# jungmannlab/picasso

Measured on AMD Instinct MI355X. Metric: localizations/sec (7x7 ROI, MLE), higher is better.
Workload: dtype f32+f64; 1 GPU; 10000-frame 512x512 uint16 simulated DNA-PAINT movie per GPU, 1001675 spots per GPU, 7x7 ROI MLE (sigmaxy), identify+cut+fit+table resident in HBM; frames=10000, height=512, width=512, box=7, max_it=100, localizations_total=1001675, mle_mode=refit, refit_spots_rank0=7346, frame_ranges_in_flight=2, all_gather=none

## Files before the change

picasso_amd/csrc/gausslq.hip:

```cpp
#include <algorithm>
#include <cstdlib>
#include <cstring>

#include "lq_common.h"

#pragma clang fp contract(off)

namespace pmi {
namespace lq {

#ifndef LQ_SBUF_PAD
#define LQ_SBUF_PAD 0
#endif
__host__ __device__ constexpr size_t lq_sbuf_doubles(int m) { return (size_t)6 * (size_t)((m + 1) & ~1) + LQ_SBUF_PAD; }
__device__ __forceinline__ void grp_sync()
{
    __builtin_amdgcn_wave_barrier();
    __threadfence_block();
    __builtin_amdgcn_wave_barrier();
}
template <int GS, int E>
__device__ __forceinline__ void rows_to_lds(const double (&v)[E], int lane, int m, double *buf)
{
#pragma unroll
// ... 721 lines not shown
    const int64_t src = (int64_t)blockIdx.x * blockDim.x + threadIdx.x;
    if (src >= n) return;
    const int64_t i = src + (d_row0 ? *d_row0 : 0);
    const float *t = th + src * 6;
    ((uint32_t *)cols.c[0])[i] = (uint32_t)frame[src];
    ((float *)cols.c[1])[i] = (float)((double)t[0] + (double)x[src]);
    ((float *)cols.c[2])[i] = (float)((double)t[1] + (double)y[src]);
    ((float *)cols.c[3])[i] = t[2];
    ((float *)cols.c[4])[i] = t[4];
    ((float *)cols.c[5])[i] = t[5];
    ((float *)cols.c[6])[i] = t[3];
    ((float *)cols.c[7])[i] = lq_precision(t[2], t[4], t[5], t[3], em);
    ((float *)cols.c[8])[i] = lq_precision(t[2], t[5], t[4], t[3], em);
    const float a = np_maxf(t[4], t[5]), b = np_minf(t[4], t[5]);
    ((float *)cols.c[9])[i] = (a - b) / a;
    ((float *)cols.c[10])[i] = ng[src];
}

}

int identify_impl(const void *d_movie, int dtype, int64_t F, int64_t Y, int64_t X, int box, double min_ng,
                  const int64_t *roi4, int64_t f_lo, int64_t f_hi, int64_t label_offset,
                  int32_t *d_frame, int32_t *d_y, int32_t *d_x, float *d_ng, int64_t cap, int64_t *d_out_n,
                  bool defer_exact, hipStream_t s);

}

extern "C" {

int pmi_gausslq_set_mode(int mode)
{
    using namespace pmi;
    if (mode != PMI_LQ_FAST && mode != PMI_LQ_REFIT && mode != PMI_LQ_STRICT) { set_error("unknown gausslq mode %d", mode); return PMI_ERR_ARG; }
    lq::g_lq_mode = mode;
    return PMI_OK;
}

int pmi_gausslq_get_mode(int *mode)
{
    if (mode) *mode = pmi::lq::lq_mode_now();
    return PMI_OK;
}

int pmi_gausslq_last_refit_count(int64_t *n_refit)
{
    unsigned h[16];
    const int rc = pmi::lq::g_lq_stats.read(h);
// ... 77 lines not shown
int pmi_localize_lq_dev(const void *d_movie, int dtype, int64_t F, int64_t Y, int64_t X, int box, double min_ng,
                        const int64_t *roi4, int64_t f_lo, int64_t f_hi, double baseline, double sensitivity,
                        double gain, int em, void *d_table, int64_t cap, int64_t *d_out_n, void *stream)
{
    using namespace pmi;
    if (cap <= 0) { set_error("capacity must be positive"); return PMI_ERR_ARG; }
    int rc = lq::check_box(box);
    if (rc != PMI_OK) return rc;
    struct Ids { int32_t *f, *y, *x; float *ng, *th; };
    auto carve = [=](void *ptr) {
        Ids d;
        d.f = (int32_t *)ptr; d.y = d.f + cap; d.x = d.y + cap;
        d.ng = (float *)(d.x + cap);
        d.th = d.ng + cap;
        return d;
    };
    lq::LqCols cols;
    for (int c = 0; c < PMI_LQ_COLUMNS; c++) cols.c[c] = (char *)d_table + (size_t)c * cap * 4;
    FusedRanges fr;
    fr.ids_bytes = (size_t)cap * (16 + 6 * 4);
    fr.capc = cap;
    fr.cap = cap;
    fr.rejects = false;
    fr.scan = [&](void *ids, int64_t lo, int64_t hi, int64_t *d_cnt, hipStream_t st) {
        const Ids d = carve(ids);
        return identify_impl(d_movie, dtype, F, Y, X, box, min_ng, roi4, lo, hi, 0, d.f, d.y, d.x, d.ng, cap, d_cnt, false, st);
    };
    fr.fit = [&](void *ids, const int64_t *d_rows, int range, hipStream_t st) {
        const Ids d = carve(ids);
        return lq::fit_movie(d_movie, dtype, Y, X, d.f, d.y, d.x, cap, d_rows, box, baseline, sensitivity, gain, d.th, nullptr,
                             nullptr, range, st);
    };
    fr.table = [&](void *ids, const int64_t *d_rows, const int64_t *d_row0, hipStream_t st) {
        const Ids d = carve(ids);
        hipLaunchKernelGGL(lq::locs_from_fits_lq_kernel, dim3((unsigned)((cap + 255) / 256)), dim3(256), 0, st, d.f, d.y, d.x, d.ng,
                           d.th, cap, d_rows, em, cols, d_row0);
        PMI_HIP(hipGetLastError());
        return PMI_OK;
    };
    return fused_ranges(fr, 1, F, Y, X, f_lo, f_hi, d_out_n, (hipStream_t)stream);
}

}
```

picasso_amd/csrc/gaussmle.hip:

```cpp
#include <algorithm>
#include <cmath>
#include <cstdlib>
#include <cstring>
#include <vector>

#include "fit_common.h"

namespace pmi {

__device__ __forceinline__ unsigned borderline(float D, int kk, float eps_lo, float eps_hi)
{
    const float wide = fmaxf(1.0f, (float)(kk - 1) * FIT_MARGIN_GROWTH);
    const float epsf = 0.5f * (eps_lo + eps_hi), epsm = 0.5f * (eps_hi - eps_lo) * wide;
    return ((D >= epsf - epsm && D < epsf + epsm) ? FLAG_MARGIN : 0u) | (kk > FIT_SLOW_ITERATIONS ? FLAG_SLOW : 0u);
}
struct StepHistory { float prev, prev2, wprev; int run; };
__device__ __forceinline__ bool wobbles(float st, float value, int kk, StepHistory &h)
{
    const float w = kk >= 3 ? (st - 2.0f * h.prev) + h.prev2 : 0.0f;
    const bool wob = w * h.wprev < 0.0f && fabsf(w) > FIT_WOBBLE_RATIO * fabsf(h.wprev) && fabsf(w) > FIT_WOBBLE_FLOOR * fabsf(value);
    h.run = wob ? h.run + 1 : 0;
    h.wprev = w; h.prev2 = h.prev; h.prev = st;
    return h.run >= FIT_WOBBLE_RUN || (h.run >= 2 && kk >= FIT_WOBBLE_LATE);
}
// ... 545 lines not shown
}

static int mle_mode_now()
{
    static const char *env = getenv("PMI_MLE_MODE");
    if (env) {
        if (!strcmp(env, "fast")) return PMI_MLE_FAST;
        if (!strcmp(env, "strict")) return PMI_MLE_STRICT;
        if (!strcmp(env, "refit")) return PMI_MLE_REFIT;
    }
    return g_mle_mode;
}
static int mle_libm_now()
{
    static const char *env = getenv("PMI_MLE_LIBM");
    if (env) {
        if (!strcmp(env, "auto")) return PMI_LIBM_AUTO;
        if (!strcmp(env, "glibc")) return PMI_LIBM_GLIBC;
        if (!strcmp(env, "device")) return PMI_LIBM_DEVICE;
    }
    return g_mle_libm;
}

int fit_impl(FitParams p, int method, bool from_movie, int range, hipStream_t s)
{
    if (p.box < 3 || p.box > PMI_MAX_BOX || (p.box & 1) == 0) { set_error("box must be odd, 3..%d (got %d)", PMI_MAX_BOX, p.box); return PMI_ERR_ARG; }
    if (method != PMI_MLE_SIGMA && method != PMI_MLE_SIGMAXY) { set_error("Method not available."); return PMI_ERR_ARG; }
    if (p.N < 0) { set_error("negative N"); return PMI_ERR_ARG; }
    if (p.N == 0) return PMI_OK;
    if (p.N > 0x7fffffffLL) { set_error("too many spots for one call"); return PMI_ERR_ARG; }
    const int g_cu_count = device_cu_count();
    const int mode = mle_mode_now();
    const int64_t BATCH = FIT_BATCH;
    const int64_t nb = (p.N + BATCH - 1) / BATCH;
    void *ptr = nullptr, *fptr = nullptr;
    int rc;
    if ((rc = scratch(SCR_FIT, (size_t)nb * 40 + 64, &ptr)) != PMI_OK) return rc;
    const size_t per_batch = (size_t)std::min<int64_t>(p.N, BATCH);
    const size_t acc_blocks = (per_batch + ACC_BLOCK - 1) / ACC_BLOCK + 2;
    if ((rc = scratch(SCR_STAGE_D, per_batch * (FISHER_STRIDE * sizeof(double) + 12 * sizeof(float) + 3 * sizeof(int32_t) + 1) + acc_blocks * sizeof(unsigned) + 32, &fptr)) != PMI_OK) return rc;
    float *state = reinterpret_cast<float *>((char *)fptr + per_batch * FISHER_STRIDE * sizeof(double));
    int32_t *flag_list = reinterpret_cast<int32_t *>(state + per_batch * 12);
    int32_t *unstable_list = flag_list + per_batch;
    int32_t *acc_list = unstable_list + per_batch;
    unsigned *acc_blk = reinterpret_cast<unsigned *>(acc_list + per_batch);
    unsigned char *refit_mark = reinterpret_cast<unsigned char *>(acc_blk + acc_blocks);
    unsigned long long *queues = (unsigned long long *)ptr;
// ... 38 lines not shown
        if (p.refit_mark && !g8) PMI_HIP(hipMemsetAsync(refit_mark, 0, (size_t)(p.N - p.first), s));
        const int64_t count = p.N - p.first;
        const int64_t blocks = std::min<int64_t>((count + FIT_WAVES - 1) / FIT_WAVES, (int64_t)g_cu_count * 8);
        const dim3 grid((unsigned)std::max<int64_t>(blocks, 1));
        auto wave_per_spot = [&](int stages) {
            p.queue = queues + 3 * bi + (stages == FIT_STAGE_FINAL ? (p.final_list ? 2 : 1) : 0);
            if (method == PMI_MLE_SIGMAXY) {
                if (from_movie) launch_fit_ppl<6, true>(ppl, grid, s, p, stages); else launch_fit_ppl<6, false>(ppl, grid, s, p, stages);
            } else {
                if (from_movie) launch_fit_ppl<5, true>(ppl, grid, s, p, stages); else launch_fit_ppl<5, false>(ppl, grid, s, p, stages);
            }
        };
        if (mode != PMI_MLE_STRICT && g8 && from_movie && cut) {
            FitParams pi = p;
            pi.spots_out = cut;
            launch_fit_g8(pi, method, true, g_cu_count, state, FIT_STAGE_INIT_ONLY, s);
            PMI_HIP(hipGetLastError());
            FitParams q = p;
            q.spots = cut - p.first * (int64_t)(p.box * p.box);
            if (p.ng_io) {
                int32_t *al = nb == 1 && p.alist_out ? p.alist_out : acc_list;
                unsigned *ab = nb == 1 && p.alist_out ? p.alist_blk_out : acc_blk;
                if ((rc = build_accept_list(p.accept, p.first, p.N, p.d_n, ab, al, s)) != PMI_OK) return rc;
                q.alist = al;
                q.alist_n = ab + (count + ACC_BLOCK - 1) / ACC_BLOCK;
            }
            launch_fit_g8(q, method, false, g_cu_count, state, FIT_STAGE_ITERATE_ONLY, s);
            PMI_HIP(hipGetLastError());
            if (mode == PMI_MLE_REFIT)
                launch_fit_strict(q, method, false, flag_list, q.flag_count, count, g_cu_count, s);
            PMI_HIP(hipGetLastError());
            launch_fit_g8(q, method, false, g_cu_count, state, FIT_STAGE_FINAL, s);
        } else {
        if (mode == PMI_MLE_STRICT) {
            FitParams ps = p;
            ps.libm_glibc = libm_all;
            launch_fit_strict(ps, method, from_movie, nullptr, nullptr, count, g_cu_count, s);
        } else {
            if (g8) launch_fit_g8(p, method, from_movie, g_cu_count, state, FIT_STAGE_NEWTON, s);
            else wave_per_spot(FIT_STAGE_NEWTON);
            PMI_HIP(hipGetLastError());
            if (mode == PMI_MLE_REFIT)
                launch_fit_strict(p, method, from_movie, flag_list, p.flag_count, count, g_cu_count, s);
        }
        PMI_HIP(hipGetLastError());
        if (g8) launch_fit_g8(p, method, from_movie, g_cu_count, state, FIT_STAGE_FINAL, s);
// ... 81 lines not shown
    ((uint32_t *)cols.c[0])[i] = (uint32_t)frame[src];
    ((float *)cols.c[1])[i] = (float)((double)t[0] + (double)x[src] - (double)off);
    ((float *)cols.c[2])[i] = (float)((double)t[1] + (double)y[src] - (double)off);
    ((float *)cols.c[3])[i] = t[2];
    ((float *)cols.c[4])[i] = t[4];
    ((float *)cols.c[5])[i] = t[5];
    ((float *)cols.c[6])[i] = t[3];
    ((float *)cols.c[7])[i] = sqrtf(c[0]);
    ((float *)cols.c[8])[i] = sqrtf(c[1]);
    float a = np_maxf(t[4], t[5]), b = np_minf(t[4], t[5]);
    ((float *)cols.c[9])[i] = (a - b) / a;
    ((float *)cols.c[10])[i] = ng[src];
    ((float *)cols.c[11])[i] = ll[src];
    ((uint32_t *)cols.c[12])[i] = (uint32_t)it[src];
    ((float *)cols.c[13])[i] = sqrtf(c[2]);
    ((float *)cols.c[14])[i] = sqrtf(c[3]);
    ((float *)cols.c[15])[i] = sqrtf(c[4]);
    ((float *)cols.c[16])[i] = sqrtf(c[5]);
}

int identify_impl(const void *d_movie, int dtype, int64_t F, int64_t Y, int64_t X, int box, double min_ng,
                  const int64_t *roi4, int64_t f_lo, int64_t f_hi, int64_t label_offset,
                  int32_t *d_frame, int32_t *d_y, int32_t *d_x, float *d_ng, int64_t cap, int64_t *d_out_n,
                  bool defer_exact, hipStream_t s);

}

extern "C" {

int pmi_mle_set_mode(int mode, double margin)
{
    using namespace pmi;
    if (mode != PMI_MLE_FAST && mode != PMI_MLE_REFIT && mode != PMI_MLE_STRICT) { set_error("unknown MLE mode %d", mode); return PMI_ERR_ARG; }
    if (!(margin >= 0.0 && margin < 1.0)) { set_error("margin must lie in [0, 1)"); return PMI_ERR_ARG; }
    g_mle_mode = mode;
    g_mle_margin = margin;
    return PMI_OK;
}

int pmi_mle_set_libm(int which)
{
    using namespace pmi;
    if (which != PMI_LIBM_DEVICE && which != PMI_LIBM_GLIBC && which != PMI_LIBM_AUTO) { set_error("unknown libm %d", which); return PMI_ERR_ARG; }
    g_mle_libm = which;
    return PMI_OK;
}

// ... 194 lines not shown
    int64_t cy0 = 0, cx0 = 0, cy1 = Y, cx1 = X;
    if (roi4) { cy0 = roi4[0]; cx0 = roi4[1]; cy1 = roi4[2]; cx1 = roi4[3]; }
    struct Ids { int32_t *f, *y, *x; float *ng, *th, *cr, *ll; int32_t *it, *tlist; unsigned *blk; unsigned char *acc; };
    const size_t acc_blocks = (size_t)((capc + ACC_BLOCK - 1) / ACC_BLOCK) + 2;
    const int nblk_c = (int)((capc + ACC_BLOCK - 1) / ACC_BLOCK);
    auto carve = [=](void *ptr) {
        Ids d;
        d.f = (int32_t *)ptr; d.y = d.f + capc; d.x = d.y + capc;
        d.ng = (float *)(d.x + capc);
        d.th = d.ng + capc; d.cr = d.th + capc * 6; d.ll = d.cr + capc * 6;
        d.it = (int32_t *)(d.ll + capc);
        d.tlist = d.it + capc;
        d.blk = (unsigned *)(d.tlist + capc);
        d.acc = (unsigned char *)(d.blk + acc_blocks);
        return d;
    };
    LocCols lc;
    for (int c = 0; c < PMI_LOC_COLUMNS; c++) lc.c[c] = (char *)d_table + (size_t)c * cap * 4;
    FusedRanges fr;
    fr.ids_bytes = (size_t)capc * (16 + 15 * 4 + 1) + acc_blocks * sizeof(unsigned) + 16;
    fr.capc = capc;
    fr.cap = cap;
    fr.rejects = defer;
    fr.scan = [&](void *ids, int64_t lo, int64_t hi, int64_t *d_cnt, hipStream_t st) {
        const Ids d = carve(ids);
        return identify_impl(d_movie, dtype, F, Y, X, box, min_ng, roi4, lo, hi, 0, d.f, d.y, d.x, d.ng, capc, d_cnt, defer, st);
    };
    fr.fit = [&](void *ids, const int64_t *d_rows, int range, hipStream_t st) {
        const Ids d = carve(ids);
        FitParams p = {};
        p.movie = d_movie; p.dtype = dtype; p.Y = Y; p.X = X; p.frame = d.f; p.y = d.y; p.x = d.x;
        p.baseline = (float)baseline; p.sensitivity = (float)sensitivity; p.gain = (float)gain; p.gdiv = make_const_div((float)gain);
        p.N = capc; p.d_n = d_rows; p.box = box; p.eps = eps; p.max_it = max_it;
        p.thetas = d.th; p.crlbs = d.cr; p.loglik = d.ll; p.iterations = d.it;
        if (defer) {
            p.ng_io = d.ng; p.accept = d.acc; p.min_ng = min_ng;
            p.crop_y0 = (int)cy0; p.crop_x0 = (int)cx0; p.crop_cy = (int)(cy1 - cy0); p.crop_cx = (int)(cx1 - cx0);
            p.alist_out = d.tlist; p.alist_blk_out = d.blk;
        }
        int r = fit_impl(p, method, true, range, st);
        if (r != PMI_OK || !defer) return r;
        if (capc <= FIT_BATCH) return PMI_OK;
        return build_accept_list(d.acc, 0, capc, d_rows, d.blk, d.tlist, st);
    };
    fr.accepted = [&](void *ids) { return (const unsigned *)(carve(ids).blk + nblk_c); };
    fr.table = [&](void *ids, const int64_t *d_rows, const int64_t *d_row0, hipStream_t st) {
        const Ids d = carve(ids);
        hipLaunchKernelGGL(locs_from_fits_kernel, dim3((unsigned)((cap + 255) / 256)), dim3(256), 0, st, d.f, d.y, d.x, d.ng, d.th,
                           d.cr, d.ll, d.it, cap, d_rows, box, lc, d_row0, (const int32_t *)(defer ? d.tlist : nullptr));
        PMI_HIP(hipGetLastError());
        return PMI_OK;
    };
    return fused_ranges(fr, 0, F, Y, X, f_lo, f_hi, d_out_n, (hipStream_t)stream);
}

}
```

picasso_amd/csrc/identify.hip:

```cpp
#include <algorithm>
#include <cmath>
#include <type_traits>
#include <mutex>
#include <vector>

#include "pmi_common.h"

#pragma clang fp contract(off)

namespace pmi {

static int64_t g_narrow_chunk_frames = 0;

static __device__ __forceinline__ float mul_rn(float a, float b) { return a * b; }
static __device__ __forceinline__ float add_rn(float a, float b) { return a + b; }
static __device__ __forceinline__ float sub_rn(float a, float b) { return a - b; }

constexpr int ID_TH = 32;
constexpr int ID_TW = 128;
constexpr int ID_NT = 256;
constexpr int ID_SHARDS = 8;

struct IdParams {
    int64_t Y, X;
// ... 314 lines not shown
        for (int k = 0; k < 4; k++) {
            if constexpr (sizeof(T) == 4 && !std::is_integral<T>::value) {
                const float f = (float)v[k];
                bad = bad || !(f >= 0.0f && f <= 65535.0f && f == __builtin_truncf(f));
                o[k] = (uint16_t)(int)f;
            } else if constexpr (std::is_signed<T>::value) {
                bad = bad || v[k] < 0 || v[k] > 65535;
                o[k] = (uint16_t)v[k];
            } else {
                bad = bad || v[k] > 65535u;
                o[k] = (uint16_t)v[k];
            }
        }
        if (full) { uint2 w; w.x = o[0] | ((unsigned)o[1] << 16); w.y = o[2] | ((unsigned)o[3] << 16); *reinterpret_cast<uint2 *>(dst + i) = w; }
        else for (int k = 0; k < 4 && i + k < n; k++) dst[i + k] = o[k];
    }
    if (__any(bad) && (threadIdx.x & 63) == 0) atomicOr(flag, 1);
}


int identify_impl(const void *d_movie, int dtype, int64_t F, int64_t Y, int64_t X, int box, double min_ng,
                  const int64_t *roi4, int64_t f_lo, int64_t f_hi, int64_t label_offset,
                  int32_t *d_frame, int32_t *d_y, int32_t *d_x, float *d_ng, int64_t cap, int64_t *d_out_n,
                  bool defer_exact, hipStream_t s)
{
    if (box < 3 || box > PMI_MAX_BOX || (box & 1) == 0) { set_error("box must be odd, 3..%d (got %d)", PMI_MAX_BOX, box); return PMI_ERR_ARG; }
    if (F < 0 || Y <= 0 || X <= 0 || Y > 65535 || X > 65535) { set_error("bad movie shape (%lld,%lld,%lld)", (long long)F, (long long)Y, (long long)X); return PMI_ERR_ARG; }
    if (cap < 0) { set_error("negative capacity"); return PMI_ERR_ARG; }
    int64_t y0 = 0, x0 = 0, y1 = Y, x1 = X;
    if (roi4) { y0 = roi4[0]; x0 = roi4[1]; y1 = roi4[2]; x1 = roi4[3]; }
    if (y0 < 0 || x0 < 0 || y1 > Y || x1 > X) { set_error("roi outside the frame"); return PMI_ERR_ARG; }
    if (f_lo < 0) f_lo = 0;
    if (f_hi > F - 1) f_hi = F - 1;
    int64_t nf = f_hi - f_lo + 1;
    int64_t cy = y1 - y0, cx = x1 - x0;

    unsigned long long *d_total = nullptr;
    void *ptr = nullptr;
    int rc;
    if ((rc = scratch(SCR_COUNTERS, 256, &ptr)) != PMI_OK) return rc;
    d_total = (unsigned long long *)ptr;
    PMI_HIP(hipMemsetAsync(d_total, 0, 256, s));
    if (nf <= 0 || cy < box + 1 || cx < box + 1) {
        PMI_HIP(hipMemsetAsync(d_out_n, 0, sizeof(int64_t), s));
        return PMI_OK;
    }
    if (nf > 0x7fffffffLL) { set_error("too many frames"); return PMI_ERR_ARG; }

    IdParams p;
    p.Y = Y; p.X = X; p.y0 = (int)y0; p.x0 = (int)x0; p.cy = (int)cy; p.cx = (int)cx;
    p.f_lo = f_lo; p.frame_label_offset = label_offset; p.nframes = (int)nf; p.box = box;
    p.tiles_y = (int)((cy + ID_TH - 1) / ID_TH); p.tiles_x = (int)((cx + ID_TW - 1) / ID_TW);
    p.min_ng = min_ng;

    const float *d_tab = nullptr;
    if ((rc = unit_table(box, &d_tab)) != PMI_OK) return rc;
    Record *recs = nullptr, *grouped = nullptr;
    int *fc = nullptr;
    size_t rec_bytes = (size_t)std::max<int64_t>(cap, 1) * sizeof(Record);
    if ((rc = scratch(SCR_RECORDS, rec_bytes * ID_SHARDS, &ptr)) != PMI_OK) return rc; recs = (Record *)ptr;
    if ((rc = scratch(SCR_RECORDS2, rec_bytes, &ptr)) != PMI_OK) return rc; grouped = (Record *)ptr;
    if ((rc = scratch(SCR_FRAME_COUNT, (size_t)nf * 3 * sizeof(int), &ptr)) != PMI_OK) return rc; fc = (int *)ptr;
    int *count = fc, *base = fc + nf, *cursor = fc + 2 * nf;
    PMI_HIP(hipMemsetAsync(count, 0, (size_t)nf * sizeof(int), s));

    {
        ScopedKernelTimer tm(s, &g_last_times.scan_ms);
        bool fast = false;
        rc = PMI_OK;
        rc = launch_scan_u16_fast(d_movie, dtype, Y, X, p.y0, p.x0, p.cy, p.cx, f_lo, label_offset, p.nframes, box, min_ng,
                                      d_tab, recs, cap, d_total, count, s, &fast, nullptr, defer_exact);
        p.gate = nullptr;
        const bool wide = dtype == PMI_U32 || dtype == PMI_I32 || dtype == PMI_F32;
        static const bool no_narrow = tuning_env("PMI_IDENTIFY_NO_NARROW") != nullptr;
        if (rc == PMI_OK && !fast && wide && !no_narrow) {
            rc = launch_scan_u16_fast(d_movie, dtype, Y, X, p.y0, p.x0, p.cy, p.cx, f_lo, label_offset, p.nframes, box, min_ng,
                                      d_tab, recs, cap, d_total, count, s, &fast, nullptr, false, (const float *)d_movie, 0);
        }
        if (rc == PMI_OK && !fast && wide && !no_narrow && ((uintptr_t)d_movie & 15) == 0 && ((Y * X) & 3) == 0) {
            const int64_t frame_px = Y * X;
            const int64_t chunk = g_narrow_chunk_frames > 0 ? g_narrow_chunk_frames : std::max<int64_t>(1, ((int64_t)1 << 29) / frame_px);
            const int64_t nchunks = (nf + chunk - 1) / chunk;
            void *tmp = nullptr, *gptr = nullptr;
            if ((rc = scratch(SCR_NARROW, (size_t)std::min<int64_t>(nf, chunk) * frame_px * 2 + 64, &tmp)) != PMI_OK) return rc;
            if ((rc = scratch(SCR_GATES, (size_t)nchunks * sizeof(int), &gptr)) != PMI_OK) return rc;
            int *gates = (int *)gptr;
            PMI_HIP(hipMemsetAsync(gates, 0, (size_t)nchunks * sizeof(int), s));
// ... 22 lines not shown
                IdParams pc = p;
                pc.f_lo = f_lo + c0; pc.nframes = (int)n; pc.gate = gates + ci;
                switch (dtype) {
                case PMI_U32: rc = launch_scan<uint32_t>(d_movie, pc, d_tab, recs, cap, d_total, count + c0, s); break;
                case PMI_I32: rc = launch_scan<int32_t>(d_movie, pc, d_tab, recs, cap, d_total, count + c0, s); break;
                default: rc = launch_scan<float>(d_movie, pc, d_tab, recs, cap, d_total, count + c0, s); break;
                }
            }
            fast = all_fast;
        }
        if (rc == PMI_OK && !fast) snprintf(g_last_scan_kernel, sizeof(g_last_scan_kernel), "identify_scan_kernel (dtype %d)", dtype);
        if (rc == PMI_OK && !fast) switch (dtype) {
        case PMI_U16: rc = launch_scan<uint16_t>(d_movie, p, d_tab, recs, cap, d_total, count, s); break;
        case PMI_U8:  rc = launch_scan<uint8_t>(d_movie, p, d_tab, recs, cap, d_total, count, s); break;
        case PMI_I16: rc = launch_scan<int16_t>(d_movie, p, d_tab, recs, cap, d_total, count, s); break;
        case PMI_U32: rc = launch_scan<uint32_t>(d_movie, p, d_tab, recs, cap, d_total, count, s); break;
        case PMI_I32: rc = launch_scan<int32_t>(d_movie, p, d_tab, recs, cap, d_total, count, s); break;
        case PMI_F32: rc = launch_scan<float>(d_movie, p, d_tab, recs, cap, d_total, count, s); break;
        default: set_error("unknown dtype code %d", dtype); rc = PMI_ERR_ARG;
        }
        tm.stop();
        if (rc != PMI_OK) return rc;
    }
    hipLaunchKernelGGL(frame_scan_kernel, dim3(1), dim3(1024), 0, s, count, base, cursor, (int)nf, d_total,
                       (long long *)d_out_n);
    if (cap > 0) {
        const unsigned sb = (unsigned)std::min<long long>((cap + 255) / 256, 512);
        hipLaunchKernelGGL(scatter_by_frame_kernel, dim3(sb, ID_SHARDS), dim3(256), 0, s, recs, d_total, (long long)cap,
                           (long long)(f_lo + label_offset), base, cursor, grouped);
        const unsigned split = (unsigned)std::min<int64_t>(16, std::max<int64_t>(1, (Y * X + 262143) / 262144));
        if (Y <= 65536 && X <= 65536)
            hipLaunchKernelGGL(sort_in_frame_kernel<true>, dim3((unsigned)nf, split), dim3(SORT_THREADS), 0, s, grouped, base,
                               count, d_total, (long long)cap, d_frame, d_y, d_x, d_ng);
        else
            hipLaunchKernelGGL(sort_in_frame_kernel<false>, dim3((unsigned)nf, split), dim3(SORT_THREADS), 0, s, grouped, base,
                               count, d_total, (long long)cap, d_frame, d_y, d_x, d_ng);
    }
    PMI_HIP(hipGetLastError());
    return PMI_OK;
}

__global__ __launch_bounds__(256) void net_gradient_kernel(const float *__restrict__ img, int Y, int X,
                                                           const int32_t *__restrict__ py, const int32_t *__restrict__ px,
                                                           int64_t n, int box, const float *__restrict__ uy,
                                                           const float *__restrict__ ux, float *__restrict__ out)
{
// ... 15 lines not shown
            const float sum = t1 + t2;
            ng = ng + sum;
        }
    }
    out[i] = ng;
}

}

extern "C" {

int pmi_identify_set_narrow_chunk(int64_t frames)
{
    if (frames < 0) { pmi::set_error("chunk length must not be negative"); return PMI_ERR_ARG; }
    pmi::g_narrow_chunk_frames = frames;
    return PMI_OK;
}

int pmi_identify_dev(const void *d_movie, int dtype, int64_t F, int64_t Y, int64_t X, int box, double min_ng,
                     const int64_t *roi4, int64_t f_lo, int64_t f_hi, int32_t *d_frame, int32_t *d_y,
                     int32_t *d_x, float *d_ng, int64_t cap, int64_t *d_out_n, void *stream)
{
    return pmi::identify_impl(d_movie, dtype, F, Y, X, box, min_ng, roi4, f_lo, f_hi, 0, d_frame, d_y, d_x, d_ng,
                              cap, d_out_n, false, (hipStream_t)stream);
}

static size_t dtype_size(int dtype)
{
    switch (dtype) {
    case PMI_U8: return 1;
    case PMI_U16: case PMI_I16: return 2;
    default: return 4;
    }
}

int pmi_identify(const void *movie, int dtype, int64_t F, int64_t Y, int64_t X, int box, double min_ng,
                 const int64_t *roi4, int64_t f_lo, int64_t f_hi, int32_t *out_frame, int32_t *out_y,
                 int32_t *out_x, float *out_ng, int64_t cap, int64_t *out_n)
{
    using namespace pmi;
    if (pmi_device_count() < 1) { set_error("no HIP device"); return PMI_ERR_NODEVICE; }
    if (!movie || !out_n) { set_error("null pointer"); return PMI_ERR_ARG; }
    if (dtype < 0 || dtype > PMI_F32) { set_error("unknown dtype code %d", dtype); return PMI_ERR_ARG; }
    if (f_lo < 0) f_lo = 0;
    if (f_hi > F - 1) f_hi = F - 1;
    *out_n = 0;
    if (f_hi < f_lo) return PMI_OK;
    const size_t frame_bytes = (size_t)Y * X * dtype_size(dtype);
    const int64_t chunk = std::max<int64_t>(1, (int64_t)((size_t)1 << 30) / (int64_t)frame_bytes);
    void *d_chunk = nullptr, *ptr = nullptr;
    int rc;
    if ((rc = scratch(SCR_STAGE_A, (size_t)std::min<int64_t>(chunk, f_hi - f_lo + 1) * frame_bytes, &d_chunk)) != PMI_OK) return rc;
    int64_t dcap = std::max<int64_t>(cap, 1);
    if ((rc = scratch(SCR_STAGE_B, (size_t)dcap * 16 + 64, &ptr)) != PMI_OK) return rc;
    int32_t *d_frame = (int32_t *)ptr, *d_y = d_frame + dcap, *d_x = d_y + dcap;
    float *d_ng = (float *)(d_x + dcap);
    int64_t *d_n = (int64_t *)(d_ng + dcap);
    int64_t total = 0;
    bool overflow = false;
    for (int64_t c0 = f_lo; c0 <= f_hi; c0 += chunk) {
        int64_t c1 = std::min(f_hi, c0 + chunk - 1), nfc = c1 - c0 + 1;
        PMI_HIP(hipMemcpy(d_chunk, (const char *)movie + (size_t)c0 * frame_bytes, (size_t)nfc * frame_bytes, hipMemcpyHostToDevice));
        int64_t room = overflow ? 0 : std::max<int64_t>(cap - total, 0);
        rc = identify_impl(d_chunk, dtype, nfc, Y, X, box, min_ng, roi4, 0, nfc - 1, c0, d_frame, d_y, d_x, d_ng,
                           room, d_n, false, nullptr);
        if (rc != PMI_OK) return rc;
        int64_t n = 0;
        PMI_HIP(hipMemcpy(&n, d_n, sizeof(n), hipMemcpyDeviceToHost));
        if (n > room) overflow = true;
        else if (n > 0) {
            PMI_HIP(hipMemcpy(out_frame + total, d_frame, (size_t)n * 4, hipMemcpyDeviceToHost));
            PMI_HIP(hipMemcpy(out_y + total, d_y, (size_t)n * 4, hipMemcpyDeviceToHost));
            PMI_HIP(hipMemcpy(out_x + total, d_x, (size_t)n * 4, hipMemcpyDeviceToHost));
            PMI_HIP(hipMemcpy(out_ng + total, d_ng, (size_t)n * 4, hipMemcpyDeviceToHost));
        }
        total += n;
    }
    *out_n = total;
    if (overflow) { set_error("identify: capacity %lld too small, %lld rows needed", (long long)cap, (long long)total); return PMI_ERR_CAPACITY; }
    return PMI_OK;
}


int pmi_net_gradient(const float *image, int64_t Y, int64_t X, const int32_t *y, const int32_t *x, int64_t n, int box,
                     const float *uy, const float *ux, float *out_ng)
{
    using namespace pmi;
    if (pmi_device_count() < 1) { set_error("no HIP device"); return PMI_ERR_NODEVICE; }
// ... 30 lines not shown
```

picasso_amd/csrc/pmi_common.h:

```cpp
#pragma once
#include <hip/hip_runtime.h>
#include <stdint.h>
#include <stdio.h>
#include <stdlib.h>
#include <string.h>

#include <functional>

#include "../../include/picasso_hip.h"

#define PMI_WAVE 64

namespace pmi {

#ifdef PMI_TUNING
inline const char *tuning_env(const char *name) { return getenv(name); }
#else
inline const char *tuning_env(const char *) { return nullptr; }
#endif

void set_error(const char *fmt, ...);
int hip_fail(hipError_t e, const char *what, const char *file, int line);

#define PMI_HIP(call)                                                          \
// ... 12 lines not shown
    SCR_RECORDS2,
    SCR_FRAME_COUNT,
    SCR_COUNTERS,
    SCR_IDS,
    SCR_FIT,
    SCR_STAGE_A,
    SCR_STAGE_B,
    SCR_STAGE_C,
    SCR_STAGE_D,
    SCR_ROWS,
    SCR_NARROW,
    SCR_GATES,
    SCR_STATS,
    SCR_LQ_STATS,
    SCR_NUM
};
int scratch(int slot, size_t bytes, void **ptr);
int scratch_release_all();
int scratch_enter_inner();
void scratch_leave_inner(int was);
unsigned scratch_generation(int slot);
unsigned scratch_generation_of(int device, int user_bank, int slot);
int scratch_user_bank();
struct SideLane { hipStream_t s2 = nullptr; hipEvent_t ev_start = nullptr, ev_scan_a = nullptr, ev_b = nullptr, stats_done[2] = {nullptr, nullptr}; };
int side_lane(int pipeline, SideLane **lane);

struct LastFitStats {
    int device = 0, bank = 0, slot = 0;
    unsigned generation = 0;
    const unsigned *buf[2] = {nullptr, nullptr};
    hipEvent_t done[2] = {nullptr, nullptr};
    int record(int pipeline, int range, const unsigned *stats, hipStream_t s);
    bool valid() const;
    int read(unsigned (&h)[16]) const;
};

struct FusedRanges {
    size_t ids_bytes;
    int64_t capc;
    int64_t cap;
    bool rejects;
    std::function<int(void *ids, int64_t f_lo, int64_t f_hi, int64_t *d_cnt, hipStream_t st)> scan;
    std::function<int(void *ids, const int64_t *d_rows, int range, hipStream_t st)> fit;
    std::function<const unsigned *(void *ids)> accepted;
    std::function<int(void *ids, const int64_t *d_rows, const int64_t *d_row0, hipStream_t st)> table;
};
int fused_ranges(const FusedRanges &c, int pipeline, int64_t F, int64_t Y, int64_t X, int64_t f_lo, int64_t f_hi,
                 int64_t *d_out_n, hipStream_t s);

struct Record {
    int32_t frame;
    uint32_t yx;
    int32_t pad;
    float ng;
};
__host__ __device__ __forceinline__ uint32_t pack_yx(int y, int x) { return ((uint32_t)y << 16) | (uint32_t)(x & 0xffff); }
constexpr uint32_t NG_DEFERRED_BITS = 0x7fc0d1feu;
extern thread_local char g_last_scan_kernel[128];
extern int g_localize_ranges;

template <typename T>
__device__ __forceinline__ float px_f32(const T *p, int64_t i) { return (float)p[i]; }

struct KernelTimes { float scan_ms, fit_ms; };
extern bool g_kernel_timing;
extern KernelTimes g_last_times;
// ... 24 lines not shown
```

picasso_amd/csrc/runtime.hip:

```cpp
#include <stdarg.h>

#include <mutex>

#include "pmi_common.h"

namespace pmi {

static thread_local char g_err[512] = "";
bool g_kernel_timing = false;
KernelTimes g_last_times = {0.f, 0.f};
int g_localize_ranges = 2;
thread_local char g_last_scan_kernel[128] = "";

void set_error(const char *fmt, ...)
{
    va_list ap;
    va_start(ap, fmt);
    vsnprintf(g_err, sizeof(g_err), fmt, ap);
    va_end(ap);
}

int hip_fail(hipError_t e, const char *what, const char *file, int line)
{
    set_error("HIP error %d (%s) in %s at %s:%d", (int)e, hipGetErrorString(e), what, file, line);
// ... 84 lines not shown
int scratch_select_bank(int bank)
{
    if (bank < 0 || bank >= SCR_USER_BANKS) { set_error("scratch bank %d out of range", bank); return PMI_ERR_ARG; }
    g_scratch_bank = bank;
    return PMI_OK;
}
int scratch_enter_inner() { const int was = g_scratch_bank; g_scratch_bank = was % SCR_USER_BANKS + SCR_USER_BANKS; return was; }
void scratch_leave_inner(int was) { g_scratch_bank = was; }

static SideLane g_side_lanes[PMI_MAX_DEVICES][SCR_USER_BANKS][2];
static std::mutex g_side_mu;
int side_lane(int pipeline, SideLane **lane)
{
    int dev = 0;
    const int rc = checked_device(&dev);
    if (rc != PMI_OK) return rc;
    std::lock_guard<std::mutex> lk(g_side_mu);
    SideLane &sd = g_side_lanes[dev][scratch_user_bank()][pipeline ? 1 : 0];
    if (!sd.s2) {
        hipStream_t s2 = nullptr;
        PMI_HIP(hipStreamCreateWithFlags(&s2, hipStreamNonBlocking));
        PMI_HIP(hipEventCreateWithFlags(&sd.ev_start, hipEventDisableTiming));
        PMI_HIP(hipEventCreateWithFlags(&sd.ev_scan_a, hipEventDisableTiming));
        PMI_HIP(hipEventCreateWithFlags(&sd.ev_b, hipEventDisableTiming));
        PMI_HIP(hipEventCreateWithFlags(&sd.stats_done[0], hipEventDisableTiming));
        PMI_HIP(hipEventCreateWithFlags(&sd.stats_done[1], hipEventDisableTiming));
        sd.s2 = s2;
    }
    *lane = &sd;
    return PMI_OK;
}

int LastFitStats::record(int pipeline, int range, const unsigned *stats, hipStream_t s)
{
    SideLane *lane = nullptr;
    const int rc = side_lane(pipeline, &lane);
    if (rc != PMI_OK) return rc;
    PMI_HIP(hipEventRecord(lane->stats_done[range], s));
    if (range == 0) buf[1] = nullptr;
    buf[range] = stats;
    done[range] = lane->stats_done[range];
    slot = pipeline ? SCR_LQ_STATS : SCR_STATS;
    device = current_device();
    bank = scratch_user_bank();
    generation = scratch_generation_of(device, bank, slot);
    return PMI_OK;
// ... 37 lines not shown
{
    const int64_t lo = f_lo < 0 ? 0 : f_lo, hi = f_hi > F - 1 ? F - 1 : f_hi, nf = hi - lo + 1;
    const bool two = g_localize_ranges == 2 && !g_kernel_timing && nf >= 16 && (double)nf * (double)Y * (double)X >= 2.5e8;
    void *ptr = nullptr, *cptr = nullptr;
    int rc;
    if ((rc = scratch(SCR_ROWS, 8 * sizeof(int64_t), &cptr)) != PMI_OK) return rc;
    int64_t *n = (int64_t *)cptr, *rows = n + 2;
    if ((rc = scratch(SCR_IDS, c.ids_bytes, &ptr)) != PMI_OK) return rc;
    void *ids[2] = {ptr, nullptr};
    auto table_rows = [&](hipStream_t st) {
        hipLaunchKernelGGL(table_rows_kernel, dim3(1), dim3(1), 0, st, (const int64_t *)n, c.rejects ? c.accepted(ids[0]) : nullptr,
                           (const int64_t *)(two ? n + 1 : nullptr), c.rejects && two ? c.accepted(ids[1]) : nullptr, c.capc,
                           c.cap, rows, d_out_n);
    };
    auto fit_rows = [&](int r, hipStream_t st) -> const int64_t * {
        if (!c.rejects && r == (two ? 1 : 0)) {
            table_rows(st);
            return rows + 2 + r;
        }
        hipLaunchKernelGGL(fit_rows_kernel, dim3(1), dim3(1), 0, st, (const int64_t *)(n + r), c.capc, rows + r);
        return rows + r;
    };
    if (!two) {
        if ((rc = c.scan(ids[0], f_lo, f_hi, n, s)) != PMI_OK) return rc;
        if ((rc = c.fit(ids[0], fit_rows(0, s), 0, s)) != PMI_OK) return rc;
    } else {
        SideLane *side_p = nullptr;
        if ((rc = side_lane(pipeline, &side_p)) != PMI_OK) return rc;
        SideLane &side = *side_p;
        const int64_t mid = lo + nf / 2 - 1;
        PMI_HIP(hipEventRecord(side.ev_start, s));
        PMI_HIP(hipStreamWaitEvent(side.s2, side.ev_start, 0));
        struct Join {
            SideLane &sd; hipStream_t st; bool done = false;
            ~Join() { if (!done) { (void)hipEventRecord(sd.ev_b, sd.s2); (void)hipStreamWaitEvent(st, sd.ev_b, 0); } }
        } join{side, s};
        if ((rc = c.scan(ids[0], lo, mid, n, s)) != PMI_OK) return rc;
        const int64_t *rows_a = fit_rows(0, s);
        PMI_HIP(hipEventRecord(side.ev_scan_a, s));
        if ((rc = c.fit(ids[0], rows_a, 0, s)) != PMI_OK) return rc;
        PMI_HIP(hipStreamWaitEvent(side.s2, side.ev_scan_a, 0));
        const int outer = scratch_enter_inner();
        rc = scratch(SCR_IDS, c.ids_bytes, &ids[1]);
        if (rc == PMI_OK) rc = c.scan(ids[1], mid + 1, hi, n + 1, side.s2);
        if (rc == PMI_OK) rc = c.fit(ids[1], fit_rows(1, side.s2), 1, side.s2);
        scratch_leave_inner(outer);
        if (rc != PMI_OK) return rc;
        PMI_HIP(hipEventRecord(side.ev_b, side.s2));
        PMI_HIP(hipStreamWaitEvent(s, side.ev_b, 0));
        join.done = true;
    }
    if (c.rejects) table_rows(s);
    if ((rc = c.table(ids[0], rows + 2, nullptr, s)) != PMI_OK) return rc;
    if (two && (rc = c.table(ids[1], rows + 3, rows + 4, s)) != PMI_OK) return rc;
    PMI_HIP(hipGetLastError());
    return PMI_OK;
}

void release_fft_plans();

}

extern "C" {

int pmi_version(void) { return 113; }

const char *pmi_last_error(void) { return pmi::g_err; }

int pmi_device_count(void)
{
    int n = 0;
    if (hipGetDeviceCount(&n) != hipSuccess) return 0;
    return n;
}

int pmi_set_device(int device)
{
// ... 81 lines not shown
```

Baseline: 375.0 million localizations/s.

## Overlap range-A table build with range-B fit using finer-grained events

Adds event hooks so the side stream can start scanning range B once range A's identify scan kernels finish, instead of waiting for the frame-count prefix scan. The main stream can then write range A's table while range B is still fitting, by waiting only on a new ev_count_b event (row count or accept list ready). The frame-count scratch is merged with the counter scratch into one memset. This adds cross-stream ordering complexity and relies on accept-list and row buffers being final when the event fires.

```diff
diff --git a/picasso_amd/csrc/gausslq.hip b/picasso_amd/csrc/gausslq.hip
--- a/picasso_amd/csrc/gausslq.hip
+++ b/picasso_amd/csrc/gausslq.hip
@@ -767,7 +767,7 @@
 int identify_impl(const void *d_movie, int dtype, int64_t F, int64_t Y, int64_t X, int box, double min_ng,
                   const int64_t *roi4, int64_t f_lo, int64_t f_hi, int64_t label_offset,
                   int32_t *d_frame, int32_t *d_y, int32_t *d_x, float *d_ng, int64_t cap, int64_t *d_out_n,
-                  bool defer_exact, hipStream_t s);
+                  bool defer_exact, hipStream_t s, hipEvent_t scanned);
 
 }
 
@@ -891,11 +891,11 @@
     fr.capc = cap;
     fr.cap = cap;
     fr.rejects = false;
-    fr.scan = [&](void *ids, int64_t lo, int64_t hi, int64_t *d_cnt, hipStream_t st) {
+    fr.scan = [&](void *ids, int64_t lo, int64_t hi, int64_t *d_cnt, hipStream_t st, hipEvent_t scanned) {
         const Ids d = carve(ids);
-        return identify_impl(d_movie, dtype, F, Y, X, box, min_ng, roi4, lo, hi, 0, d.f, d.y, d.x, d.ng, cap, d_cnt, false, st);
+        return identify_impl(d_movie, dtype, F, Y, X, box, min_ng, roi4, lo, hi, 0, d.f, d.y, d.x, d.ng, cap, d_cnt, false, st, scanned);
     };
-    fr.fit = [&](void *ids, const int64_t *d_rows, int range, hipStream_t st) {
+    fr.fit = [&](void *ids, const int64_t *d_rows, int range, hipStream_t st, hipEvent_t) {
         const Ids d = carve(ids);
         return lq::fit_movie(d_movie, dtype, Y, X, d.f, d.y, d.x, cap, d_rows, box, baseline, sensitivity, gain, d.th, nullptr,
                              nullptr, range, st);
diff --git a/picasso_amd/csrc/gaussmle.hip b/picasso_amd/csrc/gaussmle.hip
--- a/picasso_amd/csrc/gaussmle.hip
+++ b/picasso_amd/csrc/gaussmle.hip
@@ -591,7 +591,7 @@
     return g_mle_libm;
 }
 
-int fit_impl(FitParams p, int method, bool from_movie, int range, hipStream_t s)
+int fit_impl(FitParams p, int method, bool from_movie, int range, hipStream_t s, hipEvent_t counted = nullptr, bool *counted_done = nullptr)
 {
     if (p.box < 3 || p.box > PMI_MAX_BOX || (p.box & 1) == 0) { set_error("box must be odd, 3..%d (got %d)", PMI_MAX_BOX, p.box); return PMI_ERR_ARG; }
     if (method != PMI_MLE_SIGMA && method != PMI_MLE_SIGMAXY) { set_error("Method not available."); return PMI_ERR_ARG; }
@@ -676,6 +676,10 @@
                 int32_t *al = nb == 1 && p.alist_out ? p.alist_out : acc_list;
                 unsigned *ab = nb == 1 && p.alist_out ? p.alist_blk_out : acc_blk;
                 if ((rc = build_accept_list(p.accept, p.first, p.N, p.d_n, ab, al, s)) != PMI_OK) return rc;
+                if (counted && nb == 1 && p.alist_out) {
+                    PMI_HIP(hipEventRecord(counted, s));
+                    if (counted_done) *counted_done = true;
+                }
                 q.alist = al;
                 q.alist_n = ab + (count + ACC_BLOCK - 1) / ACC_BLOCK;
             }
@@ -803,7 +807,7 @@
 int identify_impl(const void *d_movie, int dtype, int64_t F, int64_t Y, int64_t X, int box, double min_ng,
                   const int64_t *roi4, int64_t f_lo, int64_t f_hi, int64_t label_offset,
                   int32_t *d_frame, int32_t *d_y, int32_t *d_x, float *d_ng, int64_t cap, int64_t *d_out_n,
-                  bool defer_exact, hipStream_t s);
+                  bool defer_exact, hipStream_t s, hipEvent_t scanned);
 
 }
 
@@ -1044,11 +1048,11 @@
     fr.capc = capc;
     fr.cap = cap;
     fr.rejects = defer;
-    fr.scan = [&](void *ids, int64_t lo, int64_t hi, int64_t *d_cnt, hipStream_t st) {
+    fr.scan = [&](void *ids, int64_t lo, int64_t hi, int64_t *d_cnt, hipStream_t st, hipEvent_t scanned) {
         const Ids d = carve(ids);
-        return identify_impl(d_movie, dtype, F, Y, X, box, min_ng, roi4, lo, hi, 0, d.f, d.y, d.x, d.ng, capc, d_cnt, defer, st);
+        return identify_impl(d_movie, dtype, F, Y, X, box, min_ng, roi4, lo, hi, 0, d.f, d.y, d.x, d.ng, capc, d_cnt, defer, st, scanned);
     };
-    fr.fit = [&](void *ids, const int64_t *d_rows, int range, hipStream_t st) {
+    fr.fit = [&](void *ids, const int64_t *d_rows, int range, hipStream_t st, hipEvent_t counted) {
         const Ids d = carve(ids);
         FitParams p = {};
         p.movie = d_movie; p.dtype = dtype; p.Y = Y; p.X = X; p.frame = d.f; p.y = d.y; p.x = d.x;
@@ -1060,10 +1064,12 @@
             p.crop_y0 = (int)cy0; p.crop_x0 = (int)cx0; p.crop_cy = (int)(cy1 - cy0); p.crop_cx = (int)(cx1 - cx0);
             p.alist_out = d.tlist; p.alist_blk_out = d.blk;
         }
-        int r = fit_impl(p, method, true, range, st);
+        bool counted_done = false;
+        int r = fit_impl(p, method, true, range, st, defer ? counted : nullptr, &counted_done);
         if (r != PMI_OK || !defer) return r;
-        if (capc <= FIT_BATCH) return PMI_OK;
-        return build_accept_list(d.acc, 0, capc, d_rows, d.blk, d.tlist, st);
+        if (capc > FIT_BATCH && (r = build_accept_list(d.acc, 0, capc, d_rows, d.blk, d.tlist, st)) != PMI_OK) return r;
+        if (counted && !counted_done) PMI_HIP(hipEventRecord(counted, st));
+        return PMI_OK;
     };
     fr.accepted = [&](void *ids) { return (const unsigned *)(carve(ids).blk + nblk_c); };
     fr.table = [&](void *ids, const int64_t *d_rows, const int64_t *d_row0, hipStream_t st) {
diff --git a/picasso_amd/csrc/identify.hip b/picasso_amd/csrc/identify.hip
--- a/picasso_amd/csrc/identify.hip
+++ b/picasso_amd/csrc/identify.hip
@@ -360,7 +360,7 @@
 int identify_impl(const void *d_movie, int dtype, int64_t F, int64_t Y, int64_t X, int box, double min_ng,
                   const int64_t *roi4, int64_t f_lo, int64_t f_hi, int64_t label_offset,
                   int32_t *d_frame, int32_t *d_y, int32_t *d_x, float *d_ng, int64_t cap, int64_t *d_out_n,
-                  bool defer_exact, hipStream_t s)
+                  bool defer_exact, hipStream_t s, hipEvent_t scanned)
 {
     if (box < 3 || box > PMI_MAX_BOX || (box & 1) == 0) { set_error("box must be odd, 3..%d (got %d)", PMI_MAX_BOX, box); return PMI_ERR_ARG; }
     if (F < 0 || Y <= 0 || X <= 0 || Y > 65535 || X > 65535) { set_error("bad movie shape (%lld,%lld,%lld)", (long long)F, (long long)Y, (long long)X); return PMI_ERR_ARG; }
@@ -376,14 +376,17 @@
     unsigned long long *d_total = nullptr;
     void *ptr = nullptr;
     int rc;
-    if ((rc = scratch(SCR_COUNTERS, 256, &ptr)) != PMI_OK) return rc;
+    const int64_t nfc = nf > 0 ? nf : 0;
+    if (nfc > 0x7fffffffLL) { set_error("too many frames"); return PMI_ERR_ARG; }
+    if ((rc = scratch(SCR_FRAME_COUNT, 256 + (size_t)nfc * 3 * sizeof(int), &ptr)) != PMI_OK) return rc;
     d_total = (unsigned long long *)ptr;
-    PMI_HIP(hipMemsetAsync(d_total, 0, 256, s));
+    int *fc = (int *)((char *)ptr + 256);
+    PMI_HIP(hipMemsetAsync(d_total, 0, 256 + (size_t)nfc * sizeof(int), s));
     if (nf <= 0 || cy < box + 1 || cx < box + 1) {
         PMI_HIP(hipMemsetAsync(d_out_n, 0, sizeof(int64_t), s));
+        if (scanned) PMI_HIP(hipEventRecord(scanned, s));
         return PMI_OK;
     }
-    if (nf > 0x7fffffffLL) { set_error("too many frames"); return PMI_ERR_ARG; }
 
     IdParams p;
     p.Y = Y; p.X = X; p.y0 = (int)y0; p.x0 = (int)x0; p.cy = (int)cy; p.cx = (int)cx;
@@ -394,13 +397,10 @@
     const float *d_tab = nullptr;
     if ((rc = unit_table(box, &d_tab)) != PMI_OK) return rc;
     Record *recs = nullptr, *grouped = nullptr;
-    int *fc = nullptr;
     size_t rec_bytes = (size_t)std::max<int64_t>(cap, 1) * sizeof(Record);
     if ((rc = scratch(SCR_RECORDS, rec_bytes * ID_SHARDS, &ptr)) != PMI_OK) return rc; recs = (Record *)ptr;
     if ((rc = scratch(SCR_RECORDS2, rec_bytes, &ptr)) != PMI_OK) return rc; grouped = (Record *)ptr;
-    if ((rc = scratch(SCR_FRAME_COUNT, (size_t)nf * 3 * sizeof(int), &ptr)) != PMI_OK) return rc; fc = (int *)ptr;
     int *count = fc, *base = fc + nf, *cursor = fc + 2 * nf;
-    PMI_HIP(hipMemsetAsync(count, 0, (size_t)nf * sizeof(int), s));
 
     {
         ScopedKernelTimer tm(s, &g_last_times.scan_ms);
@@ -469,6 +469,7 @@
         tm.stop();
         if (rc != PMI_OK) return rc;
     }
+    if (scanned) PMI_HIP(hipEventRecord(scanned, s));
     hipLaunchKernelGGL(frame_scan_kernel, dim3(1), dim3(1024), 0, s, count, base, cursor, (int)nf, d_total,
                        (long long *)d_out_n);
     if (cap > 0) {
@@ -530,7 +531,7 @@
                      int32_t *d_x, float *d_ng, int64_t cap, int64_t *d_out_n, void *stream)
 {
     return pmi::identify_impl(d_movie, dtype, F, Y, X, box, min_ng, roi4, f_lo, f_hi, 0, d_frame, d_y, d_x, d_ng,
-                              cap, d_out_n, false, (hipStream_t)stream);
+                              cap, d_out_n, false, (hipStream_t)stream, nullptr);
 }
 
 static size_t dtype_size(int dtype)
@@ -571,7 +572,7 @@
         PMI_HIP(hipMemcpy(d_chunk, (const char *)movie + (size_t)c0 * frame_bytes, (size_t)nfc * frame_bytes, hipMemcpyHostToDevice));
         int64_t room = overflow ? 0 : std::max<int64_t>(cap - total, 0);
         rc = identify_impl(d_chunk, dtype, nfc, Y, X, box, min_ng, roi4, 0, nfc - 1, c0, d_frame, d_y, d_x, d_ng,
-                           room, d_n, false, nullptr);
+                           room, d_n, false, nullptr, nullptr);
         if (rc != PMI_OK) return rc;
         int64_t n = 0;
         PMI_HIP(hipMemcpy(&n, d_n, sizeof(n), hipMemcpyDeviceToHost));
diff --git a/picasso_amd/csrc/pmi_common.h b/picasso_amd/csrc/pmi_common.h
--- a/picasso_amd/csrc/pmi_common.h
+++ b/picasso_amd/csrc/pmi_common.h
@@ -58,7 +58,7 @@
 unsigned scratch_generation(int slot);
 unsigned scratch_generation_of(int device, int user_bank, int slot);
 int scratch_user_bank();
-struct SideLane { hipStream_t s2 = nullptr; hipEvent_t ev_start = nullptr, ev_scan_a = nullptr, ev_b = nullptr, stats_done[2] = {nullptr, nullptr}; };
+struct SideLane { hipStream_t s2 = nullptr; hipEvent_t ev_start = nullptr, ev_scan_a = nullptr, ev_count_b = nullptr, ev_b = nullptr, stats_done[2] = {nullptr, nullptr}; };
 int side_lane(int pipeline, SideLane **lane);
 
 struct LastFitStats {
@@ -76,8 +76,8 @@
     int64_t capc;
     int64_t cap;
     bool rejects;
-    std::function<int(void *ids, int64_t f_lo, int64_t f_hi, int64_t *d_cnt, hipStream_t st)> scan;
-    std::function<int(void *ids, const int64_t *d_rows, int range, hipStream_t st)> fit;
+    std::function<int(void *ids, int64_t f_lo, int64_t f_hi, int64_t *d_cnt, hipStream_t st, hipEvent_t scanned)> scan;
+    std::function<int(void *ids, const int64_t *d_rows, int range, hipStream_t st, hipEvent_t counted)> fit;
     std::function<const unsigned *(void *ids)> accepted;
     std::function<int(void *ids, const int64_t *d_rows, const int64_t *d_row0, hipStream_t st)> table;
 };
diff --git a/picasso_amd/csrc/runtime.hip b/picasso_amd/csrc/runtime.hip
--- a/picasso_amd/csrc/runtime.hip
+++ b/picasso_amd/csrc/runtime.hip
@@ -130,6 +130,7 @@
         PMI_HIP(hipStreamCreateWithFlags(&s2, hipStreamNonBlocking));
         PMI_HIP(hipEventCreateWithFlags(&sd.ev_start, hipEventDisableTiming));
         PMI_HIP(hipEventCreateWithFlags(&sd.ev_scan_a, hipEventDisableTiming));
+        PMI_HIP(hipEventCreateWithFlags(&sd.ev_count_b, hipEventDisableTiming));
         PMI_HIP(hipEventCreateWithFlags(&sd.ev_b, hipEventDisableTiming));
         PMI_HIP(hipEventCreateWithFlags(&sd.stats_done[0], hipEventDisableTiming));
         PMI_HIP(hipEventCreateWithFlags(&sd.stats_done[1], hipEventDisableTiming));
@@ -213,8 +214,10 @@
         return rows + r;
     };
     if (!two) {
-        if ((rc = c.scan(ids[0], f_lo, f_hi, n, s)) != PMI_OK) return rc;
-        if ((rc = c.fit(ids[0], fit_rows(0, s), 0, s)) != PMI_OK) return rc;
+        if ((rc = c.scan(ids[0], f_lo, f_hi, n, s, nullptr)) != PMI_OK) return rc;
+        if ((rc = c.fit(ids[0], fit_rows(0, s), 0, s, nullptr)) != PMI_OK) return rc;
+        if (c.rejects) table_rows(s);
+        if ((rc = c.table(ids[0], rows + 2, nullptr, s)) != PMI_OK) return rc;
     } else {
         SideLane *side_p = nullptr;
         if ((rc = side_lane(pipeline, &side_p)) != PMI_OK) return rc;
@@ -226,24 +229,29 @@
             SideLane &sd; hipStream_t st; bool done = false;
             ~Join() { if (!done) { (void)hipEventRecord(sd.ev_b, sd.s2); (void)hipStreamWaitEvent(st, sd.ev_b, 0); } }
         } join{side, s};
-        if ((rc = c.scan(ids[0], lo, mid, n, s)) != PMI_OK) return rc;
-        const int64_t *rows_a = fit_rows(0, s);
-        PMI_HIP(hipEventRecord(side.ev_scan_a, s));
-        if ((rc = c.fit(ids[0], rows_a, 0, s)) != PMI_OK) return rc;
+        if ((rc = c.scan(ids[0], lo, mid, n, s, side.ev_scan_a)) != PMI_OK) return rc;
+        if ((rc = c.fit(ids[0], fit_rows(0, s), 0, s, nullptr)) != PMI_OK) return rc;
         PMI_HIP(hipStreamWaitEvent(side.s2, side.ev_scan_a, 0));
         const int outer = scratch_enter_inner();
         rc = scratch(SCR_IDS, c.ids_bytes, &ids[1]);
-        if (rc == PMI_OK) rc = c.scan(ids[1], mid + 1, hi, n + 1, side.s2);
-        if (rc == PMI_OK) rc = c.fit(ids[1], fit_rows(1, side.s2), 1, side.s2);
+        if (rc == PMI_OK) rc = c.scan(ids[1], mid + 1, hi, n + 1, side.s2, nullptr);
+        const int64_t *rows_b = nullptr;
+        if (rc == PMI_OK) {
+            rows_b = fit_rows(1, side.s2);
+            const hipError_t e = c.rejects ? hipSuccess : hipEventRecord(side.ev_count_b, side.s2);
+            if (e != hipSuccess) rc = hip_fail(e, "hipEventRecord(ev_count_b)", __FILE__, __LINE__);
+        }
+        if (rc == PMI_OK) rc = c.fit(ids[1], rows_b, 1, side.s2, c.rejects ? side.ev_count_b : nullptr);
         scratch_leave_inner(outer);
         if (rc != PMI_OK) return rc;
+        PMI_HIP(hipStreamWaitEvent(s, side.ev_count_b, 0));
+        if (c.rejects) table_rows(s);
+        if ((rc = c.table(ids[0], rows + 2, nullptr, s)) != PMI_OK) return rc;
         PMI_HIP(hipEventRecord(side.ev_b, side.s2));
         PMI_HIP(hipStreamWaitEvent(s, side.ev_b, 0));
         join.done = true;
-    }
-    if (c.rejects) table_rows(s);
-    if ((rc = c.table(ids[0], rows + 2, nullptr, s)) != PMI_OK) return rc;
-    if (two && (rc = c.table(ids[1], rows + 3, rows + 4, s)) != PMI_OK) return rc;
+        if ((rc = c.table(ids[1], rows + 3, rows + 4, s)) != PMI_OK) return rc;
+    }
     PMI_HIP(hipGetLastError());
     return PMI_OK;
 }
```

Measured after the change: 381.8 million localizations/s, median of 4. +1.8%, better.
